# nanoporetech/flappie

Hardware: AMD Instinct MI355X
Metric: Msamples/s basecalled (r941_native, 4k-sample chunks) (higher is better)
Workload: dtype f32 (products as 3 fp16 MFMA terms over 2-way split operands, f32 accumulate; gate activations f32 through v_exp_f32 / v_rcp_f32 with a two-word exponent and a Newton step -- FFHIP_FAST_GATES=0 replays the reference's exp_ps instead: profiles/r06_gates_c2.txt)

## Files before the change

### flappie_amd/csrc/ffhip_rnn_split.hip

```cpp
#include "ffhip_internal.hpp"
#include "ffhip_math.hpp"
#include "ffhip_split.hpp"
#include <stdlib.h>

namespace ffhip {

typedef float v4f __attribute__((ext_vector_type(4)));
typedef unsigned v4u __attribute__((ext_vector_type(4)));
typedef unsigned v2u __attribute__((ext_vector_type(2)));
typedef __bf16 v8bf __attribute__((ext_vector_type(8)));
typedef _Float16 v8h __attribute__((ext_vector_type(8)));
constexpr int NS = kSplitNS;
#ifndef FFHIP_FORCE_SKEW
#define FFHIP_FORCE_SKEW 0
#endif
#ifndef FFHIP_FORCE_RETRY
#define FFHIP_FORCE_RETRY 0
#endif

struct SplitArgs {
    const v4u *Wp;
    const float *bias;
    const unsigned char *xin;
    unsigned char *hout;
    float *hout_f32;
    unsigned *flags;
    unsigned epoch;
    unsigned *abort_word;
    int Tb, B16, H, rt0, nrt, backward, mode;
    float acc_scale;
    int scale_exp;
    int fast_gates;
    int split_gate;
    const int *tbs, *tbt;
    const unsigned *live;
    unsigned long long *dbg;
};

struct SplitArgsOther {
    const unsigned char *xin; unsigned char *hout; float *hout_f32; unsigned *flags, *abort_word; const int *tbs, *tbt; const unsigned *live; unsigned epoch; int nwg0;
};

#define RLX_AGENT __ATOMIC_RELAXED, __HIP_MEMORY_SCOPE_AGENT
#define LDSV(x) (*(volatile __attribute__((address_space(3))) int *)&(x))

template <bool CLAMP>
__device__ __forceinline__ v2u split4(v4f v, int which) {
    unsigned s[4];
    const float f[4] = { v.x, v.y, v.z, v.w };
#pragma unroll
    for (int e = 0; e < 4; e++) {
        unsigned sl[NS];
        split_slices<CLAMP>(f[e], sl);
        s[e] = sl[0];
#pragma unroll
        for (int k = 1; k < NS; k++) s[e] = (which == k) ? sl[k] : s[e];
    }
    return (v2u){ s[0] | (s[1] << 16), s[2] | (s[3] << 16) };
}

__device__ __forceinline__ v4f mm(v4u a, v4u b, v4f c) {
#ifdef FFHIP_SPLIT_BF16X3
    return __builtin_amdgcn_mfma_f32_16x16x32_bf16(__builtin_bit_cast(v8bf, a), __builtin_bit_cast(v8bf, b), c, 0, 0, 0);
#else
    return __builtin_amdgcn_mfma_f32_16x16x32_f16(__builtin_bit_cast(v8h, a), __builtin_bit_cast(v8h, b), c, 0, 0, 0);
#endif
}

template <int N, int NC = N>
__device__ __forceinline__ void mm6(const v4u (&w)[N][NC][NS], int cc, const v4u (&x)[NS], v4f (&acc)[N]) {
    constexpr int WS[kSplitNT] = FFHIP_SPLIT_TERMS_W, XS[kSplitNT] = FFHIP_SPLIT_TERMS_X;
#pragma unroll
    for (int term = 0; term < kSplitNT; term++)
#pragma unroll
        for (int j = 0; j < N; j++) acc[j] = mm(w[j][cc][WS[term]], x[XS[term]], acc[j]);
}

__device__ __forceinline__ v2u fresh_sentinel() {
    v2u v;
    asm volatile("v_mov_b32 %0, -1\n\tv_mov_b32 %1, -1" : "=v"(v.x), "=v"(v.y));
    return v;
}

__device__ __forceinline__ unsigned sentinel_max(unsigned seen, const v4u (&r)[kSplitNS]) {
#pragma unroll
    for (int s = 0; s < kSplitNS; s++) {
        seen = max(max(seen, r[s].x), r[s].y);
        seen = max(max(seen, r[s].z), r[s].w);
    }
    asm volatile("" : "+v"(seen));
    return seen;
}

__device__ __forceinline__ void wait_vmcnt_upto(int n) {
    switch (n) {
    case 0: asm volatile("s_waitcnt vmcnt(0)" ::: "memory"); break;
    case 1: asm volatile("s_waitcnt vmcnt(1)" ::: "memory"); break;
    case 2: asm volatile("s_waitcnt vmcnt(2)" ::: "memory"); break;
    case 3: asm volatile("s_waitcnt vmcnt(3)" ::: "memory"); break;
    case 4: asm volatile("s_waitcnt vmcnt(4)" ::: "memory"); break;
    case 5: asm volatile("s_waitcnt vmcnt(5)" ::: "memory"); break;
    case 6: asm volatile("s_waitcnt vmcnt(6)" ::: "memory"); break;
    case 7: asm volatile("s_waitcnt vmcnt(7)" ::: "memory"); break;
    case 8: asm volatile("s_waitcnt vmcnt(8)" ::: "memory"); break;
    case 9: asm volatile("s_waitcnt vmcnt(9)" ::: "memory"); break;
    case 10: asm volatile("s_waitcnt vmcnt(10)" ::: "memory"); break;
    case 11: asm volatile("s_waitcnt vmcnt(11)" ::: "memory"); break;
    case 12: asm volatile("s_waitcnt vmcnt(12)" ::: "memory"); break;
    default: asm volatile("s_waitcnt vmcnt(0)" ::: "memory"); break;
    }
}

template <int KIND, int N, int TS, bool DN, bool PACK = false, bool LIVE = false, int GL = 2>
__device__ __forceinline__ void lstm_split_body(const SplitArgs &a, const int block_index) {
    constexpr int fg = GL;
    static_assert(!DN || TS == 2, "the dense form is a pair form");
    static_assert(!PACK || (DN && N == 2), "the packed forms are dense forms at H = 256");
    constexpr bool PG = PACK && KIND == 1;
    constexpr int NRT = PACK ? (KIND == 1 ? 3 : 4) : N;
    constexpr int MT = PACK ? 4 : N;
    __shared__ v4f px[DN ? 1 : 2][4][TS][NRT][64];
    __shared__ v4f ph_[DN ? 1 : 4][DN ? 1 : TS][DN ? 1 : N][64];
    __shared__ int pxc[4][2];
    __shared__ v4f sbias[MT][4];
    __shared__ unsigned short gsl[8][NS][16][4];
    __shared__ float gf32[8][16][4];
    __shared__ int lds_abort;
    __shared__ int lds_fast;
    __shared__ float cx[2][64];
    __shared__ float ox[2][64];
    __shared__ int cxflag[2];
    constexpr bool HL = (TS == 1 && N == 3) || DN;
    __shared__ v4u hland[HL ? 4 : 1][HL ? TS : 1][HL ? N : 1][NS][64];
    auto ph_at = [&](int w, int ts, int j) -> v4f * {
        if constexpr (DN) return (v4f *)&hland[w][ts][0][0][0] + j * 64;
        else return &ph_[w][ts][j][0];
    };
    constexpr int G = PACK ? 16 : 32, Hc = 4 * N, Ut = 32 * N;
    constexpr size_t tileB = (size_t)Hc * NS * 1024;
    const int lane = threadIdx.x & 63;
    const int wave = __builtin_amdgcn_readfirstlane((threadIdx.x >> 6) & 7);
    const bool xw = wave < 4;
    const int kw = wave & 3;
    const int ngroup = (a.nrt + TS - 1) / TS;
    int g, m;
    {
        const int b = block_index;
        if ((ngroup & 7) == 0) { const int xcd = b & 7, j = b >> 3; g = xcd + 8 * (j / G); m = j % G; }
        else { g = b / G; m = b % G; }
    }
    const int rtA = a.rt0 + TS * g;
    const bool haveB = TS == 2 && (2 * g + 1 < a.nrt);
    const int TbA = a.tbt ? a.tbt[rtA] : a.Tb;
    const int TbB = haveB ? (a.tbt ? a.tbt[rtA + 1] : a.Tb) : 0;
    const int Tb = TbA > TbB ? TbA : TbB;
    if (Tb <= 0) return;
    const int ntl = PACK ? __builtin_amdgcn_readfirstlane((TbB > 0) ? 2 : 1) : ((TbB > 0) ? 2 : 1);
    const int ut0 = m * MT;
    if (threadIdx.x == 0) lds_abort = (__hip_atomic_load(a.abort_word, RLX_AGENT) != 0u) ? 1 : 0;
    if (threadIdx.x >= 64 && threadIdx.x < 64 + 4 * MT) sbias[(threadIdx.x - 64) >> 2][threadIdx.x & 3] = *(const v4f *)(a.bias + (size_t)ut0 * 16 + (threadIdx.x - 64) * 4) * (KIND == 1 ? 1.0f : a.acc_scale);
    const int q = lane >> 4, rl = lane & 15;
    auto step_t = [&](int i) { return a.backward ? Tb - 1 - i : i; };
    constexpr bool SGK = (KIND == 0 && N == 3 && TS == 2);
    const bool sg = SGK && ntl == 2 && a.split_gate != 0;
    const bool sg_front = sg && xw && wave < 2, sg_back = sg && xw && wave >= 2;
    const int g6 = PACK ? wave : (xw ? (sg ? 4 + (wave & 1) : 4 + wave) : kw);
    const bool gate_wave = !(sg && xw) && g6 < ntl * MT;
    const bool store_wave = gate_wave || sg_back;
    const int my_gts = g6 / MT, my_gj = g6 % MT;
    if (threadIdx.x < 2) cxflag[threadIdx.x] = 0;
    if (threadIdx.x < 8) pxc[threadIdx.x >> 1][threadIdx.x & 1] = 0;
    auto out_off = [&](int gj) { const int ut = ut0 + gj; return (unsigned)((((ut >> 3) * NS + q) * 64 + ((ut & 7) >> 1) * 16 + rl) * 16 + (ut & 1) * 8); };
    auto out_tile = [&](int t, int gts) { return a.hout + ((size_t)t * a.B16 + (rtA + gts)) * tileB; };
    auto store_wt = [&](unsigned char *tile, unsigned off, v2u v) {
        __amdgpu_buffer_rsrc_t wr = __builtin_amdgcn_make_buffer_rsrc((void *)tile, 0, (int)tileB, 0x00020000);
        __builtin_amdgcn_raw_buffer_store_b64(v, wr, off, 0, 16 );
    };
    auto store_plain = [&](unsigned char *tile, unsigned off, v2u v) {
        __amdgpu_buffer_rsrc_t wr = __builtin_amdgcn_make_buffer_rsrc((void *)tile, 0, (int)tileB, 0x00020000);
        __builtin_amdgcn_raw_buffer_store_b64(v, wr, off, 0, 0);
    };
    constexpr int AHEAD = 3;
    const v2u sentinel2 = { kSplitSentinel, kSplitSentinel };
    if (store_wave && q < NS)
        for (int k = 0; k < AHEAD && k < Tb; k++) store_wt(out_tile(step_t(k), my_gts), out_off(my_gj), sentinel2);
    __builtin_amdgcn_s_waitcnt(0x0F70);
    __syncthreads();
    if (threadIdx.x < 64) {
        unsigned xcc;
        asm volatile("s_getreg_b32 %0, hwreg(HW_REG_XCC_ID)" : "=s"(xcc));
        xcc = (a.epoch << 5) | ((xcc & 0xfu) + 1u);
        unsigned *ids = a.flags + (size_t)g * G;
        if (lane == 0) __hip_atomic_store(ids + m, xcc, RLX_AGENT);
        unsigned v = xcc;
        for (unsigned spin = 0; spin < 2000000u; spin++) {
            v = (lane < G) ? __hip_atomic_load(ids + lane, RLX_AGENT) : xcc;
            if (__all((v >> 5) == a.epoch)) break;
            __builtin_amdgcn_s_sleep(2);
        }
        if (!__all((v >> 5) == a.epoch) && lane == 0) { __hip_atomic_store(a.abort_word, 1u, RLX_AGENT); lds_abort = 1; }
        const int fast_l = (a.mode == 0 && __all(v == xcc)) ? 1 : 0;
        if (lane == 0) lds_fast = fast_l;
    }
    int chunk[N];
#pragma unroll
    for (int cc = 0; cc < N; cc++) chunk[cc] = ((kw + m) & 3) * N + (cc + (PACK ? (m >> 1) : (m >> 2))) % N;
    v4u wf[NRT][N][NS];
    {
        const v4u *wp = a.Wp + (size_t)(xw ? 0 : 1) * (PACK ? NRT * G : Ut) * Hc * NS * 64;
        const int rt_first = PACK ? NRT * m : ut0;
#pragma unroll
        for (int j = 0; j < NRT; j++)
#pragma unroll
            for (int cc = 0; cc < N; cc++)
#pragma unroll
                for (int s = 0; s < NS; s++)
                    wf[j][cc][s] = wp[(((size_t)(rt_first + j) * Hc + chunk[cc]) * NS + s) * 64 + lane];
    }
    __syncthreads();
    if (lds_abort) return;
    const bool fast = lds_fast != 0;
    if (xw) __builtin_amdgcn_s_setprio(0); else __builtin_amdgcn_s_setprio(3);

    const unsigned lane_off = (unsigned)lane * 16u;
    auto tile_ptr = [&](const unsigned char *base, int t, int ts) { return base + ((size_t)t * a.B16 + (rtA + ts)) * tileB; };
    auto raw_barrier = [&]() {
        asm volatile("s_waitcnt lgkmcnt(0)" ::: "memory");
        __builtin_amdgcn_s_barrier();
        asm volatile("" ::: "memory");
    };

#if defined(FFHIP_PHASES)
    __shared__ unsigned tl_acc[8][8];
    if (threadIdx.x < 64) tl_acc[threadIdx.x >> 3][threadIdx.x & 7] = 0u;
    unsigned tl_prev = (unsigned)__builtin_readcyclecounter();
#define TL(k) do { const unsigned now_ = (unsigned)__builtin_readcyclecounter(); if (lane == 0) __hip_atomic_fetch_add(&tl_acc[wave][(k)], now_ - tl_prev, __ATOMIC_RELAXED, __HIP_MEMORY_SCOPE_WORKGROUP); tl_prev = now_; } while (0)
#elif FFHIP_FORCE_SKEW
#define TL(k) do { if ((((unsigned)i * 5u + (unsigned)(k) * 3u + (unsigned)wave + (unsigned)m) % 13u) == 0u) __builtin_amdgcn_s_sleep(48); } while (0)
#else
#define TL(k) do { } while (0)
#endif

    const int neg_exp = -a.scale_exp;
    auto unscale4 = [&](v4f v) -> v4f { return (v4f){ __builtin_ldexpf(v.x, neg_exp), __builtin_ldexpf(v.y, neg_exp), __builtin_ldexpf(v.z, neg_exp), __builtin_ldexpf(v.w, neg_exp) }; };
    auto publish_h = [&](int i, int gts, int gj, float h) {
        const int t = step_t(i);
        unsigned lv = (unsigned)lane;
        asm volatile("" : "+v"(lv));
        const unsigned q_ = lv >> 4, rl_ = lv & 15u;
        unsigned sl_[NS];
        split_slices(h * split_pow2(kSplitExpH), sl_);
        unsigned short (*gs)[16][4] = gsl[wave];
#pragma unroll
        for (int k = 0; k < NS; k++) gs[k][rl_][q_] = (unsigned short)sl_[k];
        if (a.hout_f32) gf32[wave][rl_][q_] = h;
        asm volatile("" ::: "memory");
        const int ut = ut0 + gj;
        if (q_ < (unsigned)NS) {
            const unsigned off = (unsigned)((((ut >> 3) * NS) * 64 + ((ut & 7) >> 1) * 16) * 16 + (ut & 1) * 8) + q_ * 1024u + rl_ * 16u;
            const v2u sl = *(const v2u *)&gs[q_][rl_][0];
            unsigned char *tp_out = out_tile(t, gts);
            if (fast) {
                store_plain(tp_out, off, sl);
                if (i + AHEAD < Tb) store_plain(out_tile(step_t(i + AHEAD), gts), off, fresh_sentinel());
            } else {
                store_wt(tp_out, off, sl);
                if (i + AHEAD < Tb) store_wt(out_tile(step_t(i + AHEAD), gts), off, fresh_sentinel());
            }
        } else if (q_ == (unsigned)NS && a.hout_f32) {
            const v4f hv = *(const v4f *)&gf32[wave][rl_][0];
            __amdgpu_buffer_rsrc_t wr = __builtin_amdgcn_make_buffer_rsrc((void *)(a.hout_f32 + ((size_t)t * a.B16 + (rtA + gts)) * (size_t)(Ut * 64)), 0, Ut * 256, 0x00020000);
            __builtin_amdgcn_raw_buffer_store_b128(__builtin_bit_cast(v4u, hv), wr, rl_ * 16u, ut * 256, 0);
        }
    };
    auto gate_tile = [&](int i, int gts, int gj, float &c, int my_tb) {
        const int t = step_t(i);
        float h;
        if constexpr (PACK && KIND == 0) {
            const v4f b = sbias[gj][q];
            float s0 = b.x, s1 = b.y, s2 = b.z, s3 = b.w;
            const int rot = m + (gj >> 1);
            unsigned lv = (unsigned)lane;
            asm volatile("" : "+v"(lv));
            const char *pbase = (const char *)&hland[0][gts][0][0][0] + lv * 16u + (unsigned)gj * 4u;
#pragma unroll
            for (int w2 = 0; w2 < 4; w2++) {
                const float *pz = (const float *)(pbase + ((w2 + rot) & 3) * (int)sizeof(hland[0]));
                s0 += pz[0]; s1 += pz[64 * 4]; s2 += pz[128 * 4]; s3 += pz[192 * 4];
            }
            const v4f s = unscale4((v4f){ s0, s1, s2, s3 });
            if (fg) {
                const float forget = logistic_hw(s.y, fg) * c;
                const float update = logistic_hw(s.x, fg) * tanh_hw(s.z, fg);
                c = forget + update;
                h = logistic_hw(s.w, fg) * tanh_hw(c, fg);
            } else {
                const ffv4 L = logistic_ref4_lean((ffv4){ s.x, s.y, s.z + s.z, s.w });
                const float tanh_g = (L.z + L.z) - 1.0f;
                const float forget = L.y * c;
                const float update = L.x * tanh_g;
                c = forget + update;
                h = L.w * tanh_ref_lean(c);
            }
        } else if constexpr (PACK) {
            float sz = 0.f, sr = 0.f, su = 0.f, sx = 0.f;
            const int rot = m + (gj >> 1);
            unsigned lv = (unsigned)lane;
            asm volatile("" : "+v"(lv));
            const char *pbase = (const char *)&hland[0][gts][0][0][0] + lv * 16u + (unsigned)gj * 4u;
#pragma unroll
            for (int w2 = 0; w2 < 4; w2++) {
                const float *pz = (const float *)(pbase + ((w2 + rot) & 3) * (int)sizeof(hland[0]));
                sz += pz[0]; sr += pz[64 * 4]; su += pz[128 * 4]; sx += pz[192 * 4];
            }
            sz = __builtin_ldexpf(sz, neg_exp); sr = __builtin_ldexpf(sr, neg_exp); su = __builtin_ldexpf(su, neg_exp); sx = __builtin_ldexpf(sx, neg_exp);
            const v4f b = sbias[gj][q];
            if (fg) {
                const float z = logistic_hw(sz + b.x, fg), r = logistic_hw(sr + b.y, fg);
                const float hbar = tanh_hw(r * su + (sx + b.z), fg);
                h = z * c + (1.0f - z) * hbar;
            } else {
                const ffv2 L = logistic_ref2_lean((ffv2){ sz + b.x, sr + b.y });
                float hbar = L.y * su + (sx + b.z);
                hbar = tanh_ref_lean(hbar);
                h = L.x * c + (1.0f - L.x) * hbar;
            }
            c = h;
        } else if (KIND == 1) {
            v4f s = { 0.f, 0.f, 0.f, 0.f };
#pragma unroll
            for (int w2 = 0; w2 < 4; w2++) s = s + ph_at(w2, gts, gj)[lane];
            s = unscale4(s);
            const v4f b = sbias[gj][q];
            if (fg) {
                const float z = logistic_hw(s.x + b.x, fg), r = logistic_hw(s.y + b.y, fg);
                const float hbar = tanh_hw(r * s.z + (s.w + b.z), fg);
                h = z * c + (1.0f - z) * hbar;
            } else {
                const ffv2 L = logistic_ref2_lean((ffv2){ s.x + b.x, s.y + b.y });
                float hbar = L.y * s.z + (s.w + b.z);
                hbar = tanh_ref_lean(hbar);
                h = L.x * c + (1.0f - L.x) * hbar;
            }
            c = h;
        } else {
            v4f s = sbias[gj][q];
#pragma unroll
            for (int w2 = 0; w2 < 4; w2++) s = s + ph_at(w2, gts, gj)[lane];
            s = unscale4(s);
            if (fg) {
                const float forget = logistic_hw(s.y, fg) * c;
                const float update = logistic_hw(s.x, fg) * tanh_hw(s.z, fg);
                c = forget + update;
                h = logistic_hw(s.w, fg) * tanh_hw(c, fg);
            } else {
                const ffv4 L = logistic_ref4_lean((ffv4){ s.x, s.y, s.z + s.z, s.w });
                const float tanh_g = (L.z + L.z) - 1.0f;
                const float forget = L.y * c;
                const float update = L.x * tanh_g;
                c = forget + update;
                h = L.w * tanh_ref_lean(c);
            }
        }
        if (t >= my_tb) { h = 0.0f; c = 0.0f; }
        publish_h(i, gts, gj, h);
    };
    auto gate_front = [&](int i, int gts, int gj, float &c, int my_tb) {
        v4f s = sbias[gj][q];
#pragma unroll
        for (int w2 = 0; w2 < 4; w2++) s = s + ph_at(w2, gts, gj)[lane];
        s = unscale4(s);
        float forget, update;
        float og;
        if (fg) {
            forget = logistic_hw(s.y, fg) * c;
            update = logistic_hw(s.x, fg) * tanh_hw(s.z, fg);
            og = logistic_hw(s.w, fg);
        } else {
            const ffv4 L = logistic_ref4_lean((ffv4){ s.x, s.y, s.z + s.z, s.w });
            const float tanh_g = (L.z + L.z) - 1.0f;
            forget = L.y * c;
            update = L.x * tanh_g;
            og = L.w;
        }
        ox[wave & 1][lane] = og;
        c = forget + update;
        if (step_t(i) >= my_tb) c = 0.0f;
        cx[wave & 1][lane] = c;
        asm volatile("s_waitcnt lgkmcnt(0)" ::: "memory");
        if (lane == 0) LDSV(cxflag[wave & 1]) = i + 1;
    };
    auto gate_back = [&](int i, int gts, int gj, int my_tb) {
        while (LDSV(cxflag[wave & 1]) != i + 1) __builtin_amdgcn_s_sleep(1);
        asm volatile("" ::: "memory");
        const float c = cx[wave & 1][lane];
        const float o = ox[wave & 1][lane];
        float h = o * (fg ? tanh_hw(c, fg) : tanh_ref_lean(c));
        if (step_t(i) >= my_tb) h = 0.0f;
        publish_h(i, gts, gj, h);
    };
    int my_tb = 0;
    if (gate_wave || sg_front || sg_back) my_tb = a.tbs ? a.tbs[(rtA + my_gts) * 16 + rl] : a.Tb;
    float c = 0.0f;
    auto live_word = [&](int i) -> unsigned {
        unsigned w = 0u;
        if constexpr (LIVE) {
            const unsigned *lp = a.live + ((size_t)step_t(i) * a.B16 + (rtA + my_gts));
            asm volatile("s_load_dword %0, %1, 0x0\n\ts_waitcnt lgkmcnt(0)" : "=s"(w) : "s"(lp) : "memory");
        }
        return w;
    };
    auto tb_of = [&](unsigned w) -> int {
        if constexpr (!LIVE) return my_tb;
        unsigned lv = (unsigned)lane;
        asm volatile("" : "+v"(lv));
        return ((w >> (lv & 15u)) & 1u) ? 0x7fffffff : 0;
    };

    if (xw && DN) {
        if constexpr (DN) {
        v4u xb[N][NS];
        auto load_x_tile = [&](int i, int ts) {
            __amdgpu_buffer_rsrc_t rx = __builtin_amdgcn_make_buffer_rsrc((void *)tile_ptr(a.xin, step_t(i), ts), 0, (int)tileB, 0x00020000);
#pragma unroll
            for (int cc = 0; cc < N; cc++) {
#pragma unroll
                for (int s = 0; s < NS; s++) xb[cc][s] = __builtin_amdgcn_raw_buffer_load_b128(rx, lane_off, ((chunk[cc] * NS + s) * 64) * 16, 0);
                if (cc + 1 < N) __builtin_amdgcn_s_sleep(1);
            }
        };
        constexpr int XPRE = KIND == 1 ? 2 : 1;
        constexpr bool XP = PACK || (KIND == 0 && N == 3);
        v4u xq[2][NS];
        auto ldq = [&](int i, int k, v4u (&dst)[NS]) {
            const int ts = (k / N < ntl) ? k / N : 0, cc = k % N;
            __amdgpu_buffer_rsrc_t rx = __builtin_amdgcn_make_buffer_rsrc((void *)tile_ptr(a.xin, step_t(i), ts), 0, (int)tileB, 0x00020000);
#pragma unroll
            for (int s = 0; s < NS; s++) dst[s] = __builtin_amdgcn_raw_buffer_load_b128(rx, lane_off, ((chunk[cc] * NS + s) * 64) * 16, 0);
        };
        auto project_step = [&](int i, int want) {
            v4f acc[TS][NRT];
            if constexpr (XP) {
                if constexpr (XPRE < 1) ldq(i, 0, xq[0]);
                if constexpr (XPRE < 2) ldq(i, 1, xq[1]);
#pragma unroll
                for (int ts = 0; ts < TS; ts++)
#pragma unroll
                    for (int j = 0; j < NRT; j++) acc[ts][j] = (v4f){ 0.f, 0.f, 0.f, 0.f };
#pragma unroll
                for (int k = 0; k < TS * N; k++) {
                    mm6<NRT, N>(wf, k % N, xq[k & 1], acc[k / N]);
                    __builtin_amdgcn_sched_barrier(0);
                    if (k + 2 < TS * N) ldq(i, k + 2, xq[k & 1]);
                    else if (k + 2 - TS * N < XPRE) ldq(i + 1 < Tb ? i + 1 : i, k + 2 - TS * N, xq[k & 1]);
                    __builtin_amdgcn_sched_barrier(0);
                }
            } else
#pragma unroll
            for (int ts = 0; ts < TS; ts++) {
                if (ts >= ntl) continue;
                if constexpr (!(PACK && KIND == 0)) load_x_tile(i, ts);
#pragma unroll
                for (int j = 0; j < NRT; j++) acc[ts][j] = (v4f){ 0.f, 0.f, 0.f, 0.f };
                if constexpr (PACK && KIND == 0) {
                    __amdgpu_buffer_rsrc_t rx = __builtin_amdgcn_make_buffer_rsrc((void *)tile_ptr(a.xin, step_t(i), ts), 0, (int)tileB, 0x00020000);
#pragma unroll
                    for (int cc = 0; cc < N; cc++) {
#pragma unroll
                        for (int s = 0; s < NS; s++) xb[0][s] = __builtin_amdgcn_raw_buffer_load_b128(rx, lane_off, ((chunk[cc] * NS + s) * 64) * 16, 0);
                        mm6<NRT, N>(wf, cc, xb[0], acc[ts]);
                        __builtin_amdgcn_sched_barrier(0);
                    }
                } else {
#pragma unroll
                for (int cc = 0; cc < N; cc++) mm6<NRT, N>(wf, cc, xb[cc], acc[ts]);
                }
            }
#pragma unroll
            for (int ts = 0; ts < TS; ts++) {
                if (ts >= ntl) continue;
                if (want > 0)
                    for (unsigned spin = 0; LDSV(pxc[kw][ts]) != want && 0 == LDSV(lds_abort) && spin < 40000000u; spin++) __builtin_amdgcn_s_sleep(1);
#pragma unroll
                for (int j = 0; j < NRT; j++) px[0][kw][ts][j][lane] = acc[ts][j];
            }
        };
        constexpr int WARM = 3;
        constexpr int LPM = (Hc * NS * 8 * TS + G - 1) / G;
        unsigned touched = 0, sink = 0;
        auto touch_x = [&](int i) {
            unsigned lt = (unsigned)lane;
            if constexpr (XP && KIND == 0) asm volatile("" : "+v"(lt));
            const int line = m * LPM + (int)lt;
            unsigned t = 0;
            if (wave == 3 && lane < LPM && line < ntl * Hc * NS * 8 && i < Tb)
                t = *(const unsigned *)(tile_ptr(a.xin, step_t(i), 0) + (size_t)line * 128);
            touched = t;
        };
        if constexpr (XP) { if constexpr (XPRE >= 1) ldq(0, 0, xq[0]); if constexpr (XPRE >= 2) ldq(0, 1, xq[1]); }
        project_step(0, 0);
        touch_x(1);
        sink ^= touched;
        touch_x(2);
        raw_barrier();
        for (int i = 0; i < Tb; i++) {
            TL(0);
            const unsigned lw = live_word(i);
            if (i + 1 < Tb) project_step(i + 1, i + 1);
            sink ^= touched;
            touch_x(i + WARM);
            TL(2);
            raw_barrier();
            TL(3);
            const int aborted = LDSV(lds_abort);
            if (sg_front) {
                __builtin_amdgcn_s_setprio(3);
                gate_front(i, my_gts, my_gj, c, tb_of(lw));
                __builtin_amdgcn_s_setprio(0);
            } else if (sg_back) {
                __builtin_amdgcn_s_setprio(3);
                gate_back(i, my_gts, my_gj, tb_of(lw));
                __builtin_amdgcn_s_setprio(0);
            } else if (gate_wave) {
                if (PACK) __builtin_amdgcn_s_setprio(3);
                gate_tile(i, my_gts, my_gj, c, tb_of(lw));
                if (PACK) __builtin_amdgcn_s_setprio(0);
            }
            if (aborted) return;
            TL(4);
            raw_barrier();
            TL(5);
        }
        if (sink == 0x9e3779b9u && a.Tb < 0) a.flags[0] = sink;
        }
    } else if (xw) {
        v4u xb[TS][N][NS];
        auto load_x = [&](int i) {
            const int t = step_t(i);
#pragma unroll
            for (int ts = 0; ts < TS; ts++) {
                if (ts >= ntl) continue;
                const v4u *p = (const v4u *)(tile_ptr(a.xin, t, ts) + lane_off);
#pragma unroll
                for (int cc = 0; cc < N; cc++) {
#pragma unroll
                    for (int s = 0; s < NS; s++) xb[ts][cc][s] = p[(chunk[cc] * NS + s) * 64];
                    __builtin_amdgcn_s_sleep(2);
                }
            }
        };
        auto project = [&](int i) {
#pragma unroll
            for (int ts = 0; ts < TS; ts++) {
                if (ts >= ntl) continue;
                v4f acc[N];
#pragma unroll
                for (int j = 0; j < N; j++) acc[j] = (v4f){ 0.f, 0.f, 0.f, 0.f };
#pragma unroll
                for (int cc = 0; cc < N; cc++)
                    if constexpr (!PACK) mm6<N>(wf, cc, xb[ts][cc], acc);
#pragma unroll
                for (int j = 0; j < N; j++) px[DN ? 0 : (i & 1)][kw][ts][j][lane] = acc[j];
            }
        };
        constexpr int WARM = 3;
        constexpr int LPM = (Hc * NS * 8 * TS + 31) / 32;
        unsigned touched = 0, sink = 0;
        auto touch_x = [&](int i) {
            const int line = m * LPM + lane;
            unsigned t = 0;
            if (wave == 3 && lane < LPM && line < ntl * Hc * NS * 8 && i < Tb)
                t = *(const unsigned *)(tile_ptr(a.xin, step_t(i), 0) + (size_t)line * 128);
            touched = t;
        };
        load_x(0);
        project(0);
        if (Tb > 1) load_x(1);
        touch_x(2);
        raw_barrier();
        for (int i = 0; i < Tb; i++) {
            TL(0);
            const unsigned lw = live_word(i);
            if (i + 1 < Tb) {
                project(i + 1);
                if (i + 2 < Tb) load_x(i + 2);
            }
            sink ^= touched;
            touch_x(i + WARM);
            TL(2);
            raw_barrier();
            TL(3);
            const int aborted = LDSV(lds_abort);
            if constexpr (TS == 2) {
                if (sg_front) {
                    __builtin_amdgcn_s_setprio(3);
                    gate_front(i, my_gts, my_gj, c, tb_of(lw));
                    __builtin_amdgcn_s_setprio(0);
                } else if (sg_back) gate_back(i, my_gts, my_gj, tb_of(lw));
                else if (gate_wave) gate_tile(i, my_gts, my_gj, c, tb_of(lw));
            }
            if (aborted) return;
            TL(4);
            raw_barrier();
            TL(5);
        }
        if (sink == 0x9e3779b9u && a.Tb < 0) a.flags[0] = sink;
    } else {
        constexpr int NPROD = 8 * N;
        constexpr int NCH = TS * N;
        raw_barrier();
        for (int i = 0; i < Tb; i++) {
            TL(0);
            const unsigned lw = live_word(i);
            v4f acc[TS][N];
            auto init_acc = [&]() {
#pragma unroll
                for (int ts = 0; ts < TS; ts++)
#pragma unroll
                    for (int j = 0; j < N; j++) {
                        const v4f p = px[DN ? 0 : (i & 1)][kw][ts][j][lane];
                        acc[ts][j] = KIND == 1 ? (v4f){ p.x, p.y, 0.0f, p.z } : p;
                    }
            };
            if constexpr (!DN) init_acc();
            v4f pc[PG ? 2 : 1][3];
            if constexpr (PG) {
#pragma unroll
                for (int ts = 0; ts < 2; ts++)
#pragma unroll
                    for (int j = 0; j < 3; j++) pc[ts][j] = px[0][kw][ts][j][lane];
                asm volatile("s_waitcnt lgkmcnt(0)" ::: "memory");
                if (lane < 2) LDSV(pxc[kw][lane]) = i + 1;
            }
            if (i > 0) {
                const int tp = step_t(i - 1);
                const unsigned char *hp = tile_ptr(a.hout, tp, 0);
                __amdgpu_buffer_rsrc_t rs2 = __builtin_amdgcn_make_buffer_rsrc((void *)hp, 0, (int)(TS * tileB), 0x00020000);
                bool timed_out = false;
                {
                    const int ul = lane % NPROD, pts = lane / NPROD;
                    const int put = ((kw + m) & 3) * NPROD + ul;
                    const bool act = pts < ntl;
                    const unsigned poff = (unsigned)(pts * (int)tileB + ((put >> 3) * NS * 64 + ((put & 7) >> 1) * 16 + 15) * 16 + (put & 1) * 8);
                    for (unsigned spin = 0; ; spin++) {
                        const unsigned v = act ? __builtin_amdgcn_raw_buffer_load_b32(rs2, poff, 0, 16 ) : 0u;
                        if (__all(v != kSplitSentinel)) break;
                        if (spin > 6000000u || (spin & 511u) == 511u) {
                            const unsigned ab = __hip_atomic_load(a.abort_word, RLX_AGENT);
                            if (ab != 0u || spin > 6000000u) { timed_out = true; break; }
                        }
                    }
                }
                TL(1);
                v4u raw[NCH][NS];
                const int offB = (TS > 1 && ntl > 1) ? (int)tileB : 0;
                auto load_chunk = [&](int k) {
                    const int ts = k / N, cc = k % N;
#pragma unroll
                    for (int s = 0; s < NS; s++) {
                        raw[k][s] = __builtin_amdgcn_raw_buffer_load_b128(rs2, ts * offB + ((chunk[cc] * NS + s) * 64) * 16 + lane_off, 0, 16 );
                    }
                };
                auto recur = [&]() -> bool {
                    bool ok = true;
#pragma unroll
                    for (int k = 0; k < NCH; k++) {
                        load_chunk(k);
                        if (k + 1 < NCH) __builtin_amdgcn_s_sleep(1);
                    }
#pragma unroll
                    for (int k = 0; k < NCH; k++) {
#pragma unroll
                        for (int s = 0; s < NS; s++) {
                            const v4u r = raw[k][s];
                            ok = ok && r.x != kSplitSentinel && r.y != kSplitSentinel && r.z != kSplitSentinel && r.w != kSplitSentinel;
                        }
                        if constexpr (!PACK) mm6<N>(wf, k % N, raw[k], acc[k / N]);
                        __builtin_amdgcn_sched_barrier(0);
                    }
                    return __all(ok) != 0;
                };
                auto recur_lds = [&]() -> bool {
                    unsigned seen = 0u;
#if defined(__HIP_DEVICE_COMPILE__)
                    if constexpr (HL && !DN) {
#pragma unroll
                        for (int k = 0; k < N; k++) {
#pragma unroll
                            for (int s = 0; s < NS; s++)
                                __builtin_amdgcn_raw_ptr_buffer_load_lds(rs2, (__attribute__((address_space(3))) void *)&hland[kw][0][k][s][0], 16,
                                                                         lane_off, ((chunk[k] * NS + s) * 64) * 16, 0, 16 );
                            if (k + 1 < N) __builtin_amdgcn_s_sleep(1);
                        }
                        const unsigned la = (unsigned)(size_t)(__attribute__((address_space(3))) void *)&hland[kw][0][0][0][lane];
                        v4u r[2][NS];
                        auto fetch = [&](int k) {
                            wait_vmcnt_upto(NS * (N - 1 - k));
                            asm volatile("ds_read_b128 %0, %2\n\tds_read_b128 %1, %2 offset:1024"
                                         : "=&v"(r[k & 1][0]), "=&v"(r[k & 1][1]) : "v"(la + (unsigned)(k * NS * 1024)) : "memory");
                        };
                        fetch(0);
#pragma unroll
                        for (int k = 0; k < N; k++) {
                            asm volatile("s_waitcnt lgkmcnt(0)" : "+v"(r[k & 1][0]), "+v"(r[k & 1][1]) :: "memory");
                            if (k + 1 < N) fetch(k + 1);
                            seen = sentinel_max(seen, r[k & 1]);
                            if constexpr (!PACK) mm6<N>(wf, k, r[k & 1], acc[0]);
                            __builtin_amdgcn_sched_barrier(0);
                        }
                    }
#endif
                    return __all(seen != kSplitSentinel) != 0;
                };
                auto recur_dn = [&]() -> bool {
                    unsigned seen = 0u;
#if defined(__HIP_DEVICE_COMPILE__)
                    if constexpr (DN) {
#pragma unroll
                        for (int ts = 0; ts < 2; ts++)
#pragma unroll
                            for (int k = 0; k < N; k++) {
#pragma unroll
                                for (int s = 0; s < NS; s++)
                                    __builtin_amdgcn_raw_ptr_buffer_load_lds(rs2, (__attribute__((address_space(3))) void *)&hland[kw][ts][k][s][0], 16,
                                                                             lane_off, ts * offB + ((chunk[k] * NS + s) * 64) * 16, 0, 16 );
                                if (ts * N + k + 1 < 2 * N) __builtin_amdgcn_s_sleep(1);
                            }
                        const unsigned la = (unsigned)(size_t)(__attribute__((address_space(3))) void *)&hland[kw][0][0][0][lane];
                        v4u r[2][NS];
                        auto fetch = [&](int c) {
                            wait_vmcnt_upto(NS * (2 * N - 1 - c));
                            asm volatile("ds_read_b128 %0, %2\n\tds_read_b128 %1, %2 offset:1024"
                                         : "=&v"(r[c & 1][0]), "=&v"(r[c & 1][1]) : "v"(la + (unsigned)(c * NS * 1024)) : "memory");
                        };
                        fetch(0);
#pragma unroll
                        for (int ts = 0; ts < 2; ts++) {
                            v4f accd[NRT], xc = { 0.f, 0.f, 0.f, 0.f };
                            if constexpr (PACK && KIND == 0) {
#pragma unroll
                                for (int j = 0; j < NRT; j++) accd[j] = px[0][kw][ts][j][lane];
                            } else if constexpr (PACK) {
                                accd[0] = pc[ts][0]; accd[1] = pc[ts][1]; accd[2] = (v4f){ 0.f, 0.f, 0.f, 0.f }; xc = pc[ts][2];
                            } else {
#pragma unroll
                                for (int j = 0; j < N; j++) {
                                    const v4f p = px[0][kw][ts][j][lane];
                                    accd[j] = KIND == 1 ? (v4f){ p.x, p.y, 0.0f, p.z } : p;
                                }
                            }
#pragma unroll
                            for (int k = 0; k < N; k++) {
                                const int c = ts * N + k;
                                asm volatile("s_waitcnt lgkmcnt(0)" : "+v"(r[c & 1][0]), "+v"(r[c & 1][1]) :: "memory");
                                if (c + 1 < 2 * N) fetch(c + 1);
                                seen = sentinel_max(seen, r[c & 1]);
                                mm6<NRT, N>(wf, k, r[c & 1], accd);
                                __builtin_amdgcn_sched_barrier(0);
                            }
                            if (ts < ntl) {
#pragma unroll
                                for (int j = 0; j < NRT; j++) ph_at(kw, ts, j)[lane] = accd[j];
                                if constexpr (PG) ph_at(kw, ts, 3)[lane] = xc;
                            }
                        }
                    }
#endif
                    return __all(seen != kSplitSentinel) != 0;
                };
                auto recur_any = [&]() -> bool { if constexpr (DN) return recur_dn(); else if constexpr (HL) return recur_lds(); else return recur(); };
                if (!timed_out) {
                    __builtin_amdgcn_s_waitcnt(0x0F70);
                    if (!recur_any() || (FFHIP_FORCE_RETRY && (i & 31) == 5)) {
                        for (unsigned spin = 0;; spin++) {
                            if (spin > 3000000u || (spin & 255u) == 255u) {
                                const unsigned ab = __hip_atomic_load(a.abort_word, RLX_AGENT);
                                if (ab != 0u || spin > 3000000u) { timed_out = true; break; }
                            }
                            __builtin_amdgcn_s_sleep(1);
                            asm volatile("s_waitcnt vmcnt(0) lgkmcnt(0)" ::: "memory");
                            if constexpr (!DN) init_acc();
                            if (recur_any()) break;
                        }
                    }
                }
                if (timed_out && lane == 0) { __hip_atomic_store(a.abort_word, 1u, RLX_AGENT); lds_abort = 1; }
            }
            if constexpr (DN) {
                if (i == 0) {
                    if constexpr (PACK && KIND == 0) {
#pragma unroll
                        for (int ts = 0; ts < TS; ts++) {
                            if (ts >= ntl) continue;
#pragma unroll
                            for (int j = 0; j < NRT; j++) ph_at(kw, ts, j)[lane] = px[0][kw][ts][j][lane];
                        }
                    } else if constexpr (PACK) {
#pragma unroll
                        for (int ts = 0; ts < TS; ts++) {
                            if (ts >= ntl) continue;
                            ph_at(kw, ts, 0)[lane] = pc[ts][0];
                            ph_at(kw, ts, 1)[lane] = pc[ts][1];
                            ph_at(kw, ts, 2)[lane] = (v4f){ 0.f, 0.f, 0.f, 0.f };
                            ph_at(kw, ts, 3)[lane] = pc[ts][2];
                        }
                    } else {
                    init_acc();
#pragma unroll
                    for (int ts = 0; ts < TS; ts++) {
                        if (ts >= ntl) continue;
#pragma unroll
                        for (int j = 0; j < N; j++) ph_at(kw, ts, j)[lane] = acc[ts][j];
                    }
                    }
                }
                asm volatile("s_waitcnt lgkmcnt(0)" ::: "memory");
                if (!PG && lane < 2) LDSV(pxc[kw][lane]) = i + 1;
            } else {
#pragma unroll
                for (int ts = 0; ts < TS; ts++) {
                    if (ts >= ntl) continue;
#pragma unroll
                    for (int j = 0; j < N; j++) ph_at(kw, ts, j)[lane] = acc[ts][j];
                }
            }
            TL(2);
            raw_barrier();
            TL(3);
            const int aborted = LDSV(lds_abort);
            if (gate_wave) gate_tile(i, my_gts, my_gj, c, tb_of(lw));
            if (aborted) return;
            TL(4);
            __builtin_amdgcn_s_barrier();
            asm volatile("" ::: "memory");
            TL(5);
        }
    }
#ifdef FFHIP_PHASES
    asm volatile("s_waitcnt lgkmcnt(0)" ::: "memory");
    if (a.dbg && lane < 8) {
        atomicAdd(a.dbg + wave * 8 + lane, (unsigned long long)tl_acc[wave][lane]);
        if (lane == 0) atomicAdd(a.dbg + 64 + wave, (unsigned long long)Tb);
    }
#endif
}

template <int KIND, int N, int TS, bool DN = false, bool LIVE = false, int GL = 2>
__global__ void __launch_bounds__(512, (DN && N <= 2) ? 6 : ((TS == 1 || N <= 2 || DN) ? 4 : 1))
k_lstm_split(SplitArgs a) { lstm_split_body<KIND, N, TS, DN, false, LIVE, GL>(a, (int)blockIdx.x); }

template <bool LIVE, int GL>
__global__ void __launch_bounds__(512, 4)
k_grumod_pack(SplitArgs a) { lstm_split_body<1, 2, 2, true, true, LIVE, GL>(a, (int)blockIdx.x); }
template <bool LIVE, int GL>
__global__ void __launch_bounds__(512, 4)
k_lstm_pack(SplitArgs a) { lstm_split_body<0, 2, 2, true, true, LIVE, GL>(a, (int)blockIdx.x); }

template <int KIND, int N, int TS, bool DN, bool LIVE = false, int GL = 2>
__global__ void __launch_bounds__(512, (DN && N <= 2) ? 6 : ((TS == 1 || N <= 2 || DN) ? 4 : 1))
k_lstm_split_pair(SplitArgs a, SplitArgsOther o) {
    int bi = (int)blockIdx.x;
    if (bi >= o.nwg0) {
        bi -= o.nwg0;
        a.xin = o.xin; a.hout = o.hout; a.hout_f32 = o.hout_f32; a.flags = o.flags; a.abort_word = o.abort_word; a.tbs = o.tbs; a.tbt = o.tbt; a.live = o.live; a.epoch = o.epoch;
    }
    lstm_split_body<KIND, N, TS, DN, false, LIVE, GL>(a, bi);
}

struct RnnSplitArgs {
    const v4u *Wp;
    const v4f *xa;
    unsigned char *hout;
    float *hout_f32;
    unsigned *flags, *abort_word;
    int Tb, B16, rt0, nrt, backward, mode;
    float acc_scale;
    const int *tbs, *tbt;
};

template <int N, int CPW>
__global__ void __launch_bounds__(512, 1)
k_rnn_split(RnnSplitArgs a) {
    constexpr int G = 32, Hc = 8 * CPW, Ut = 32 * N, NCH = 2 * CPW, NPROD = 8 * CPW;
    constexpr size_t tileB = (size_t)Hc * NS * 1024;
    __shared__ v4f ph[8][2][N][64];
    __shared__ unsigned short gsl[8][NS][16][4];
    __shared__ float gf32[8][16][4];
    __shared__ int lds_abort;
    __shared__ int lds_fast;
    const int lane = threadIdx.x & 63;
    const int wave = __builtin_amdgcn_readfirstlane(threadIdx.x >> 6);
    const int ngroup = (a.nrt + 1) >> 1;
    int g, m;
    {
        const int b = blockIdx.x;
        if ((ngroup & 7) == 0) { const int xcd = b & 7, j = b >> 3; g = xcd + 8 * (j / G); m = j % G; }
        else { g = b / G; m = b % G; }
    }
    const int rtA = a.rt0 + 2 * g;
    const bool haveB = (2 * g + 1 < a.nrt);
    const int TbA = a.tbt ? a.tbt[rtA] : a.Tb;
    const int TbB = haveB ? (a.tbt ? a.tbt[rtA + 1] : a.Tb) : 0;
    const int Tb = TbA > TbB ? TbA : TbB;
    if (Tb <= 0) return;
    const int ntl = (TbB > 0) ? 2 : 1;
    const int ut0 = m * N;
    if (threadIdx.x == 0) lds_abort = (__hip_atomic_load(a.abort_word, RLX_AGENT) != 0u) ? 1 : 0;
    const int q = lane >> 4, rl = lane & 15;
    auto step_t = [&](int i) { return a.backward ? Tb - 1 - i : i; };
    const bool gate_wave = wave < ntl * N;
    const int my_gts = wave / N, my_gj = wave % N;
    auto out_off = [&](int gj) { const int ut = ut0 + gj; return (unsigned)((((ut >> 3) * NS + q) * 64 + ((ut & 7) >> 1) * 16 + rl) * 16 + (ut & 1) * 8); };
    auto out_tile = [&](int t, int gts) { return a.hout + ((size_t)t * a.B16 + (rtA + gts)) * tileB; };
    auto store_wt = [&](unsigned char *tile, unsigned off, v2u v) {
        __amdgpu_buffer_rsrc_t wr = __builtin_amdgcn_make_buffer_rsrc((void *)tile, 0, (int)tileB, 0x00020000);
        __builtin_amdgcn_raw_buffer_store_b64(v, wr, off, 0, 16 );
    };
    constexpr int AHEAD = 3;
    const v2u sentinel2 = { kSplitSentinel, kSplitSentinel };
    if (gate_wave && q < NS)
        for (int k = 0; k < AHEAD && k < Tb; k++) store_wt(out_tile(step_t(k), my_gts), out_off(my_gj), sentinel2);
    __builtin_amdgcn_s_waitcnt(0x0F70);
    __syncthreads();
    if (threadIdx.x < 64) {
        unsigned xcc;
        asm volatile("s_getreg_b32 %0, hwreg(HW_REG_XCC_ID)" : "=s"(xcc));
        xcc = (xcc & 0xfu) + 1u;
        unsigned *ids = a.flags + (size_t)g * G;
        if (lane == 0) __hip_atomic_store(ids + m, xcc, RLX_AGENT);
        unsigned v = xcc;
        for (unsigned spin = 0; spin < 2000000u; spin++) {
            v = (lane < G) ? __hip_atomic_load(ids + lane, RLX_AGENT) : xcc;
            if (__all(v != 0u)) break;
            __builtin_amdgcn_s_sleep(2);
        }
        if (!__all(v != 0u) && lane == 0) { __hip_atomic_store(a.abort_word, 1u, RLX_AGENT); lds_abort = 1; }
        const int fast_l = (a.mode == 0 && __all(v == xcc)) ? 1 : 0;
        if (lane == 0) lds_fast = fast_l;
    }
    const int cbase = ((wave + m) & 7) * CPW;
    v4u wf[N][CPW][NS];
#pragma unroll
    for (int j = 0; j < N; j++)
#pragma unroll
        for (int cc = 0; cc < CPW; cc++)
#pragma unroll
            for (int s = 0; s < NS; s++)
                wf[j][cc][s] = a.Wp[(((size_t)(ut0 + j) * Hc + (cbase + cc)) * NS + s) * 64 + lane];
    __syncthreads();
    if (lds_abort) return;
    const bool fast = lds_fast != 0;
    const unsigned lane_off = (unsigned)lane * 16u;
    auto raw_barrier = [&]() {
        asm volatile("s_waitcnt lgkmcnt(0)" ::: "memory");
        __builtin_amdgcn_s_barrier();
        asm volatile("" ::: "memory");
    };
    int my_tb = 0;
    if (gate_wave) my_tb = a.tbs ? a.tbs[(rtA + my_gts) * 16 + rl] : a.Tb;
    float c = 0.0f;
    auto xa_tile = [&](int i) { return a.xa[(((size_t)step_t(i) * a.B16 + (rtA + my_gts)) * Ut + ut0 + my_gj) * 64 + lane]; };
    v4f xa_next = gate_wave ? xa_tile(0) : (v4f){ 0.f, 0.f, 0.f, 0.f };
    for (int i = 0; i < Tb; i++) {
        v4f acc[2][N];
#pragma unroll
        for (int ts = 0; ts < 2; ts++)
#pragma unroll
            for (int j = 0; j < N; j++) acc[ts][j] = (v4f){ 0.f, 0.f, 0.f, 0.f };
        const v4f xa_cur = xa_next;
        if (i > 0) {
            const int tp = step_t(i - 1);
            const unsigned char *hp = a.hout + ((size_t)tp * a.B16 + rtA) * tileB;
            __amdgpu_buffer_rsrc_t rs2 = __builtin_amdgcn_make_buffer_rsrc((void *)hp, 0, (int)(2 * tileB), 0x00020000);
            bool timed_out = false;
            {
                const int ul = lane % NPROD, pts = lane / NPROD;
                const int put = cbase * 8 + ul;
                const bool act = pts < ntl;
                const unsigned poff = (unsigned)(pts * (int)tileB + ((put >> 3) * NS * 64 + ((put & 7) >> 1) * 16 + 15) * 16 + (put & 1) * 8);
                for (unsigned spin = 0;; spin++) {
                    const unsigned v = act ? __builtin_amdgcn_raw_buffer_load_b32(rs2, poff, 0, 16 ) : 0u;
                    if (__all(v != kSplitSentinel)) break;
                    if (spin > 6000000u || (spin & 511u) == 511u) {
                        const unsigned ab = __hip_atomic_load(a.abort_word, RLX_AGENT);
                        if (ab != 0u || spin > 6000000u) { timed_out = true; break; }
                    }
                }
            }
            v4u raw[NCH][NS];
            const int offB = (ntl > 1) ? (int)tileB : 0;
            auto recur = [&]() -> bool {
                bool ok = true;
#pragma unroll
                for (int k = 0; k < NCH; k++) {
#pragma unroll
                    for (int s = 0; s < NS; s++)
                        raw[k][s] = __builtin_amdgcn_raw_buffer_load_b128(rs2, (k / CPW) * offB + (((cbase + k % CPW) * NS + s) * 64) * 16 + lane_off, 0, 16 );
                    if (k + 1 < NCH) __builtin_amdgcn_s_sleep(1);
                }
#pragma unroll
                for (int k = 0; k < NCH; k++) {
#pragma unroll
                    for (int s = 0; s < NS; s++) {
                        const v4u r = raw[k][s];
                        ok = ok && r.x != kSplitSentinel && r.y != kSplitSentinel && r.z != kSplitSentinel && r.w != kSplitSentinel;
                    }
                    mm6<N, CPW>(wf, k % CPW, raw[k], acc[k / CPW]);
                    __builtin_amdgcn_sched_barrier(0);
                }
                return __all(ok) != 0;
            };
            if (!timed_out) {
                __builtin_amdgcn_s_waitcnt(0x0F70);
                if (!recur()) {
                    for (unsigned spin = 0;; spin++) {
                        if (spin > 3000000u || (spin & 255u) == 255u) {
                            const unsigned ab = __hip_atomic_load(a.abort_word, RLX_AGENT);
                            if (ab != 0u || spin > 3000000u) { timed_out = true; break; }
                        }
                        __builtin_amdgcn_s_sleep(1);
#pragma unroll
                        for (int ts = 0; ts < 2; ts++)
#pragma unroll
                            for (int j = 0; j < N; j++) acc[ts][j] = (v4f){ 0.f, 0.f, 0.f, 0.f };
                        if (recur()) break;
                    }
                }
            }
            if (timed_out && lane == 0) { __hip_atomic_store(a.abort_word, 1u, RLX_AGENT); lds_abort = 1; }
        }
        if (gate_wave && i + 1 < Tb) xa_next = xa_tile(i + 1);
#pragma unroll
        for (int ts = 0; ts < 2; ts++) {
            if (ts >= ntl) continue;
#pragma unroll
            for (int j = 0; j < N; j++) ph[wave][ts][j][lane] = acc[ts][j];
        }
        raw_barrier();
        if (lds_abort) return;
        if (gate_wave) {
            const int t = step_t(i);
            v4f s = xa_cur * a.acc_scale;
            if (i > 0) {
#pragma unroll
                for (int w2 = 0; w2 < 8; w2++) s = s + ph[w2][my_gts][my_gj][lane];
            }
            s = s * (1.0f / a.acc_scale);
            const ffv4 L = logistic_ref4_lean((ffv4){ s.x, s.y, s.z + s.z, s.w });
            const float tanh_g = (L.z + L.z) - 1.0f;
            const float forget = L.y * c;
            const float update = L.x * tanh_g;
            c = forget + update;
            float h = L.w * tanh_ref_lean(c);
            if (t >= my_tb) { h = 0.0f; c = 0.0f; }
            {
                unsigned sl[NS];
                split_slices(h * split_pow2(kSplitExpH), sl);
#pragma unroll
                for (int k = 0; k < NS; k++) gsl[wave][k][rl][q] = (unsigned short)sl[k];
            }
            if (a.hout_f32) gf32[wave][rl][q] = h;
            asm volatile("" ::: "memory");
            const int ut = ut0 + my_gj;
            const unsigned off = out_off(my_gj);
            if (q < NS) {
                const v2u sl = *(const v2u *)&gsl[wave][q][rl][0];
                unsigned char *tp_out = out_tile(t, my_gts);
                if (fast) {
                    *(v2u *)(tp_out + off) = sl;
                    if (i + AHEAD < Tb) *(v2u *)(out_tile(step_t(i + AHEAD), my_gts) + off) = sentinel2;
                } else {
                    store_wt(tp_out, off, sl);
                    if (i + AHEAD < Tb) store_wt(out_tile(step_t(i + AHEAD), my_gts), off, sentinel2);
                }
            } else if (a.hout_f32) {
                const v4f hv = *(const v4f *)&gf32[wave][rl][0];
                *(v4f *)(a.hout_f32 + ((size_t)t * a.B16 + (rtA + my_gts)) * (size_t)(Ut * 64) + (size_t)ut * 64 + rl * 4) = hv;
            }
        }
        __builtin_amdgcn_s_barrier();
        asm volatile("" ::: "memory");
    }
}

bool rnn_split_supported(int kind, int H) { return kind == 0 && (H == 256 || H == 512); }
bool launch_rnn_split(hipStream_t s, const void *Wsplit, const float *xa, void *hout, float *hout_f32, unsigned *flags, unsigned *abort_word,
                      int Tb, int B16, int H, int rt0, int nrt, int backward, int mode, int scale_exp, const int *tbs, const int *tbt) {
    RnnSplitArgs a;
    a.acc_scale = split_pow2(scale_exp);
    const int Ut = H / 4, Hc = H / 32;
    a.Wp = (const v4u *)Wsplit + (size_t)Ut * Hc * NS * 64;
    a.xa = (const v4f *)xa; a.hout = (unsigned char *)hout; a.hout_f32 = hout_f32; a.flags = flags; a.abort_word = abort_word;
    a.Tb = Tb; a.B16 = B16; a.rt0 = rt0; a.nrt = nrt; a.backward = backward; a.mode = mode; a.tbs = tbs; a.tbt = tbt;
    const int ngroup = (nrt + 1) / 2;
    if (H == 512) { hipLaunchKernelGGL((k_rnn_split<4, 2>), dim3(ngroup * 32), dim3(512), 0, s, a); return true; }
    if (H == 256) { hipLaunchKernelGGL((k_rnn_split<2, 1>), dim3(ngroup * 32), dim3(512), 0, s, a); return true; }
    return false;
}

__global__ void __launch_bounds__(256)
k_inproj_split(const unsigned char *__restrict__ in, float *__restrict__ xa, const v4u *__restrict__ Wp, const float *__restrict__ bias,
               int ntile, int Mt, int Hc, float acc_scale) {
    constexpr int TM = 4, TN = 6;
    const int lane = threadIdx.x & 63, wave = threadIdx.x >> 6;
    const int wm = wave & 1, wn = wave >> 1;
    const int nMblk = (Mt + 2 * TM - 1) / (2 * TM);
    const int nNblk = (ntile + 2 * TN - 1) / (2 * TN);
    const int L = blockIdx.x;
    const int mblk = L % nMblk, nblk = L / nMblk;
    if (nblk >= nNblk) return;
    const int mt0 = (mblk * 2 + wm) * TM, nt0 = (nblk * 2 + wn) * TN;
    const int kq = lane >> 4;
    v4f acc[TM][TN];
    const v4u *ap[TM], *bp[TN];
#pragma unroll
    for (int i = 0; i < TM; i++) {
        const int mt = min(mt0 + i, Mt - 1);
        ap[i] = Wp + (size_t)mt * Hc * NS * 64 + lane;
        const v4f bv = *(const v4f *)(bias + mt * 16 + kq * 4) * acc_scale;
#pragma unroll
// ... 328 lines not shown
```

Baseline: 120.6.

## Replace px spin-flag handshake with barrier-ordered write in dense non-packed form

For the dense, non-packed kernel variant, the projection waves now compute the next step's input projection into registers before the barrier and write it to the px LDS buffer only after the barrier. This removes the per-step pxc counter spin-wait and the matching lgkmcnt wait and flag store on the recurrent waves. It also raises wave priority across the px write and the gate phase. The cost is holding the accumulator registers live across the barrier, which adds register pressure, and the ordering now depends on barrier placement rather than explicit flags.

```diff
diff --git a/flappie_amd/csrc/ffhip_rnn_split.hip b/flappie_amd/csrc/ffhip_rnn_split.hip
--- a/flappie_amd/csrc/ffhip_rnn_split.hip
+++ b/flappie_amd/csrc/ffhip_rnn_split.hip
@@ -131,6 +131,7 @@
     __shared__ float ox[2][64];
     __shared__ int cxflag[2];
     constexpr bool HL = (TS == 1 && N == 3) || DN;
+    constexpr bool PXB = DN && !PACK;
     __shared__ v4u hland[HL ? 4 : 1][HL ? TS : 1][HL ? N : 1][NS][64];
     auto ph_at = [&](int w, int ts, int j) -> v4f * {
         if constexpr (DN) return (v4f *)&hland[w][ts][0][0][0] + j * 64;
@@ -169,7 +170,7 @@
     const bool store_wave = gate_wave || sg_back;
     const int my_gts = g6 / MT, my_gj = g6 % MT;
     if (threadIdx.x < 2) cxflag[threadIdx.x] = 0;
-    if (threadIdx.x < 8) pxc[threadIdx.x >> 1][threadIdx.x & 1] = 0;
+    if constexpr (!PXB) { if (threadIdx.x < 8) pxc[threadIdx.x >> 1][threadIdx.x & 1] = 0; }
     auto out_off = [&](int gj) { const int ut = ut0 + gj; return (unsigned)((((ut >> 3) * NS + q) * 64 + ((ut & 7) >> 1) * 16 + rl) * 16 + (ut & 1) * 8); };
     auto out_tile = [&](int t, int gts) { return a.hout + ((size_t)t * a.B16 + (rtA + gts)) * tileB; };
     auto store_wt = [&](unsigned char *tile, unsigned off, v2u v) {
@@ -438,8 +439,7 @@
 #pragma unroll
             for (int s = 0; s < NS; s++) dst[s] = __builtin_amdgcn_raw_buffer_load_b128(rx, lane_off, ((chunk[cc] * NS + s) * 64) * 16, 0);
         };
-        auto project_step = [&](int i, int want) {
-            v4f acc[TS][NRT];
+        auto project_mm = [&](int i, v4f (&acc)[TS][NRT]) {
             if constexpr (XP) {
                 if constexpr (XPRE < 1) ldq(i, 0, xq[0]);
                 if constexpr (XPRE < 2) ldq(i, 1, xq[1]);
@@ -476,11 +476,15 @@
                 for (int cc = 0; cc < N; cc++) mm6<NRT, N>(wf, cc, xb[cc], acc[ts]);
                 }
             }
+        };
+        auto write_px = [&](const v4f (&acc)[TS][NRT], int want) {
 #pragma unroll
             for (int ts = 0; ts < TS; ts++) {
                 if (ts >= ntl) continue;
-                if (want > 0)
-                    for (unsigned spin = 0; LDSV(pxc[kw][ts]) != want && 0 == LDSV(lds_abort) && spin < 40000000u; spin++) __builtin_amdgcn_s_sleep(1);
+                if constexpr (PACK) {
+                    if (want > 0)
+                        for (unsigned spin = 0; LDSV(pxc[kw][ts]) != want && 0 == LDSV(lds_abort) && spin < 40000000u; spin++) __builtin_amdgcn_s_sleep(1);
+                }
 #pragma unroll
                 for (int j = 0; j < NRT; j++) px[0][kw][ts][j][lane] = acc[ts][j];
             }
@@ -498,15 +502,57 @@
             touched = t;
         };
         if constexpr (XP) { if constexpr (XPRE >= 1) ldq(0, 0, xq[0]); if constexpr (XPRE >= 2) ldq(0, 1, xq[1]); }
-        project_step(0, 0);
+        {
+            v4f acc0[TS][NRT];
+            project_mm(0, acc0);
+            write_px(acc0, 0);
+        }
         touch_x(1);
         sink ^= touched;
         touch_x(2);
         raw_barrier();
+        if constexpr (PXB) {
         for (int i = 0; i < Tb; i++) {
             TL(0);
             const unsigned lw = live_word(i);
-            if (i + 1 < Tb) project_step(i + 1, i + 1);
+            const bool more = i + 1 < Tb;
+            v4f acc[TS][NRT];
+            if (more) project_mm(i + 1, acc);
+            else {
+#pragma unroll
+                for (int ts = 0; ts < TS; ts++)
+#pragma unroll
+                    for (int j = 0; j < NRT; j++) acc[ts][j] = (v4f){ 0.f, 0.f, 0.f, 0.f };
+            }
+            TL(6);
+            sink ^= touched;
+            touch_x(i + WARM);
+            TL(2);
+            raw_barrier();
+            TL(3);
+            __builtin_amdgcn_s_setprio(3);
+            if (more) write_px(acc, 0);
+            __builtin_amdgcn_sched_barrier(0);
+            TL(7);
+            const int aborted = LDSV(lds_abort);
+            if (sg_front) gate_front(i, my_gts, my_gj, c, tb_of(lw));
+            else if (sg_back) gate_back(i, my_gts, my_gj, tb_of(lw));
+            else if (gate_wave) gate_tile(i, my_gts, my_gj, c, tb_of(lw));
+            __builtin_amdgcn_s_setprio(0);
+            if (aborted) return;
+            TL(4);
+            raw_barrier();
+            TL(5);
+        }
+        } else
+        for (int i = 0; i < Tb; i++) {
+            TL(0);
+            const unsigned lw = live_word(i);
+            if (i + 1 < Tb) {
+                v4f acc[TS][NRT];
+                project_mm(i + 1, acc);
+                write_px(acc, i + 1);
+            }
             sink ^= touched;
             touch_x(i + WARM);
             TL(2);
@@ -814,8 +860,10 @@
                     }
                     }
                 }
-                asm volatile("s_waitcnt lgkmcnt(0)" ::: "memory");
-                if (!PG && lane < 2) LDSV(pxc[kw][lane]) = i + 1;
+                if constexpr (PACK) {
+                    asm volatile("s_waitcnt lgkmcnt(0)" ::: "memory");
+                    if (!PG && lane < 2) LDSV(pxc[kw][lane]) = i + 1;
+                }
             } else {
 #pragma unroll
                 for (int ts = 0; ts < TS; ts++) {
```

Measured after the change: 122.9, median of 6. 1.02x the previous value.
